# LiliMeng/network_interpretation_imagenet

Measured on NVIDIA B200. Metric: masked forward evals/sec (ResNet-101 224^2), higher is better.
Workload: dtype bf16

## Files before the change

network_interpretation_imagenet_b200/classifier.py:

```python
from __future__ import annotations

import ctypes as C

import numpy as np
import torch
import torch.nn as nn

from . import _lib


def _f32(t: torch.Tensor) -> np.ndarray:
    return np.ascontiguousarray(t.detach().to(torch.float32).cpu().numpy())


def fold_bn(conv_w: torch.Tensor, conv_b: torch.Tensor | None, bn: nn.BatchNorm2d | None):
    w = conv_w.detach().double()
    b = conv_b.detach().double() if conv_b is not None else torch.zeros(w.shape[0], dtype=torch.float64, device=w.device)
    if bn is not None:
        scale = bn.weight.detach().double() / torch.sqrt(bn.running_var.detach().double() + bn.eps)
        w = w * scale.view(-1, 1, 1, 1)
        b = bn.bias.detach().double() + (b - bn.running_mean.detach().double()) * scale
    elif conv_b is None:
        return w.float(), None
    return w.float(), b.float()
# ... 204 lines not shown
        buf = self.taps[name]
        H, W, Cc = C.c_int(), C.c_int(), C.c_int()
        _lib.check(self.lib.nib_net_buffer_info(self.h, buf, None, C.byref(H), C.byref(W), C.byref(Cc), None, None),
                   "nib_net_buffer_info")
        out = torch.empty(N, Cc.value, H.value, W.value, dtype=torch.float32, device="cuda")
        _lib.check(self.lib.nib_net_read_buffer_nchw(self.h, buf, N, out.data_ptr(), _lib.stream_handle()),
                   "nib_net_read_buffer_nchw")
        return out


def _in_cpad(Cin: int) -> int:
    return 4 if Cin <= 4 else Cin


def _lower_tv_resnet(m, hw, prec, precision, max_batch):
    H, W = hw
    b = _Builder(prec, max_batch)
    cin = m.conv1.in_channels
    c1 = m.conv1
    stem_tc = (precision == "bf16" and c1.kernel_size == (7, 7) and c1.stride == (2, 2) and c1.padding == (3, 3) and cin <= 8)
    split = precision == "split"
    x_in = (b.buffer(H, W, 4 if cin <= 4 else 8, pad=3, pooled=False) if stem_tc
            else b.buffer(H, W, _in_cpad(cin), pooled=False, f32=split))
    Hc, Wc = _out_hw(H, c1.kernel_size[0], c1.stride[0], c1.padding[0]), _out_hw(W, c1.kernel_size[0], c1.stride[0], c1.padding[0])
    t = b.buffer(Hc, Wc, c1.out_channels, f32=split)
    w, bias = fold_bn(c1.weight, c1.bias, m.bn1)
    b.conv(x_in, cin, t, c1.out_channels, w, bias, c1.kernel_size[0], c1.stride[0], c1.padding[0], relu=True)
    mp = m.maxpool
    k, s, p = mp.kernel_size, mp.stride, mp.padding
    Hp, Wp = _out_hw(Hc, k, s, p), _out_hw(Wc, k, s, p)
    x = b.buffer(Hp, Wp, c1.out_channels, f32=split)
    b.pool(_lib.POOL_MAX, t, c1.out_channels, x, k, s, p)
    b.release(t)
    if split:
        xs = b.buffer(Hp, Wp, c1.out_channels)
        b.convert(x, xs)
        b.release(x)
        x = xs
    Cx, Hx, Wx = c1.out_channels, Hp, Wp
    for layer in (m.layer1, m.layer2, m.layer3, m.layer4):
        for blk in layer:
            convs = [(blk.conv1, blk.bn1), (blk.conv2, blk.bn2)]
            if hasattr(blk, "conv3"):
                convs.append((blk.conv3, blk.bn3))
            if blk.downsample is not None:
                dc, dbn = blk.downsample[0], blk.downsample[1]
                Hd, Wd = _out_hw(Hx, dc.kernel_size[0], dc.stride[0], dc.padding[0]), _out_hw(Wx, dc.kernel_size[0], dc.stride[0], dc.padding[0])
                idn = b.buffer(Hd, Wd, dc.out_channels)
                w, bias = fold_bn(dc.weight, dc.bias, dbn)
                b.conv(x, Cx, idn, dc.out_channels, w, bias, dc.kernel_size[0], dc.stride[0], dc.padding[0], relu=False)
            else:
                idn = x
            cur, Cc, Hh, Ww = x, Cx, Hx, Wx
            tmp = []
            for i, (cv, bn) in enumerate(convs):
                last = i == len(convs) - 1
                Ho, Wo = _out_hw(Hh, cv.kernel_size[0], cv.stride[0], cv.padding[0]), _out_hw(Ww, cv.kernel_size[0], cv.stride[0], cv.padding[0])
                o = b.buffer(Ho, Wo, cv.out_channels)
                w, bias = fold_bn(cv.weight, cv.bias, bn)
                if last:
                    b.conv(cur, Cc, o, cv.out_channels, w, bias, cv.kernel_size[0], cv.stride[0], cv.padding[0],
                           relu=True, res=idn, res_C=cv.out_channels)
                else:
                    b.conv(cur, Cc, o, cv.out_channels, w, bias, cv.kernel_size[0], cv.stride[0], cv.padding[0], relu=True)
                    tmp.append(o)
                cur, Cc, Hh, Ww = o, cv.out_channels, Ho, Wo
            for tbuf in tmp:
                b.release(tbuf)
            if idn != x:
                b.release(idn)
            b.release(x)
            x, Cx, Hx, Wx = cur, Cc, Hh, Ww
    if split:
        xf = b.buffer(Hx, Wx, Cx, f32=True)
        b.convert(x, xf)
        x = xf
    feat = b.buffer(1, 1, Cx, f32=split)
    assert Hx == Wx, "global average pool expects a square map"
    b.pool(_lib.POOL_AVG, x, Cx, feat, Hx, Hx, 0)
    b.fc(feat, Cx, m.fc.out_features, m.fc.weight, m.fc.bias)
    return Classifier(b, x_in, (cin, H, W), m.fc.out_features, precision, max_batch, arch="tv_resnet")


def _lower_resnet_cifar(m, hw, prec, precision, max_batch):
    H, W = hw
    b = _Builder(prec, max_batch)
    cp = (lambda c: max(c, 64)) if precision == "bf16" else (lambda c: c)

    def padw(w, bias, co, ci):
        if co == w.shape[0] and ci == w.shape[1]:
            return w, bias
        wp = torch.zeros(co, ci, w.shape[2], w.shape[3], dtype=w.dtype, device=w.device)
        wp[:w.shape[0], :w.shape[1]] = w
        bp = None
        if bias is not None:
            bp = torch.zeros(co, dtype=bias.dtype, device=bias.device)
            bp[:bias.shape[0]] = bias
        return wp, bp

    x_in = b.buffer(H, W, _in_cpad(3), pooled=False)
    x = b.buffer(H, W, cp(16))
    w, bias = padw(*fold_bn(m.conv1.weight, None, m.bn1), cp(16), 3)
    b.conv(x_in, 3, x, cp(16), w, bias, 3, 1, 1, relu=True)
    Cx, Hx, Wx = 16, H, W
    for layer in (m.layer1, m.layer2, m.layer3):
        for blk in layer:
            s = blk.conv1.stride[0]
            planes = blk.conv1.out_channels
            Ho, Wo = _out_hw(Hx, 3, s, 1), _out_hw(Wx, 3, s, 1)
            t = b.buffer(Ho, Wo, cp(planes))
            w, bias = padw(*fold_bn(blk.conv1.weight, None, blk.bn1), cp(planes), cp(Cx))
            b.conv(x, cp(Cx), t, cp(planes), w, bias, 3, s, 1, relu=True)
            if blk.downsample is not None:
                ks = blk.downsample.avg.kernel_size
# ... 67 lines not shown
            b.release(mid)
            cur += c2.out_channels
        else:
            b.conv(blk_buf, cur, blk_buf, c1.out_channels, c1.weight.detach().float(), None, 3, 1, 1, relu=False,
                   out_coff=cur, pre=bn_affine(n1))
            cur += c1.out_channels
    assert cur == Ctot
    return cur


def _lower_tv_densenet(m, hw, prec, precision, max_batch):
    H, W = hw
    f = m.features
    b = _Builder(prec, max_batch)
    c0 = f.conv0
    stem_tc = (precision == "bf16" and c0.kernel_size == (7, 7) and c0.stride == (2, 2) and c0.padding == (3, 3))
    x_in = b.buffer(H, W, 4, pad=3, pooled=False) if stem_tc else b.buffer(H, W, _in_cpad(3), pooled=False)
    Hc, Wc = _out_hw(H, 7, 2, 3), _out_hw(W, 7, 2, 3)
    t = b.buffer(Hc, Wc, c0.out_channels)
    w, bias = fold_bn(c0.weight, None, f.norm0)
    b.conv(x_in, 3, t, c0.out_channels, w, bias, 7, 2, 3, relu=True)
    Hx, Wx = _out_hw(Hc, 3, 2, 1), _out_hw(Wc, 3, 2, 1)
    blocks = [getattr(f, n) for n in ("denseblock1", "denseblock2", "denseblock3", "denseblock4")]
    trans = [getattr(f, n) for n in ("transition1", "transition2", "transition3")]
    Cin = c0.out_channels
    prev, prev_is_stem = t, True
    for bi, blk in enumerate(blocks):
        layers = list(blk.children())
        growth = layers[0].conv2.out_channels
        Ctot = Cin + growth * len(layers)
        buf = b.buffer(Hx, Wx, Ctot, pooled=False)
        if prev_is_stem:
            b.pool(_lib.POOL_MAX, prev, Cin, buf, 3, 2, 1)
            b.release(prev)
        else:
            b.pool(_lib.POOL_AVG, prev, Cin, buf, 2, 2, 0)
            b.release(prev)
        _dense_block(b, layers, buf, Cin, Hx, Wx, Ctot)
        if bi < len(trans):
            tr = trans[bi]
            Co = tr.conv.out_channels
            tt = b.buffer(Hx, Wx, Co)
            b.conv(buf, Ctot, tt, Co, tr.conv.weight.detach().float(), None, 1, 1, 0, relu=False, pre=bn_affine(tr.norm))
            prev, prev_is_stem = tt, False
            Cin = Co
            Hx, Wx = Hx // 2, Wx // 2
        else:
            feat = b.buffer(1, 1, Ctot)
            assert Hx == Wx
            b.pool(_lib.POOL_AVG, buf, Ctot, feat, Hx, Hx, 0, pre=bn_affine(f.norm5))
            b.fc(feat, Ctot, m.classifier.out_features, m.classifier.weight, m.classifier.bias)
    return Classifier(b, x_in, (3, H, W), m.classifier.out_features, precision, max_batch, arch="tv_densenet")


def _lower_densenet_cifar(m, hw, prec, precision, max_batch):
    H, W = hw
    b = _Builder(prec, max_batch)
    x_in = b.buffer(H, W, _in_cpad(3), pooled=False)
    seq = list(m.blocks.children())
    Cin = m.stem.out_channels
    Hx, Wx = H, W
    prev = None
    for i in range(0, len(seq), 2):
        layers = list(seq[i].children())
        growth = (layers[0].conv2 if hasattr(layers[0], "conv2") else layers[0].conv1).out_channels
        Ctot = Cin + growth * len(layers)
        buf = b.buffer(Hx, Wx, Ctot, pooled=False)
        if prev is None:
            b.conv(x_in, 3, buf, Cin, m.stem.weight.detach().float(), None, 3, 1, 1, relu=False)
        else:
            b.pool(_lib.POOL_AVG, prev, Cin, buf, 2, 2, 0)
            b.release(prev)
        _dense_block(b, layers, buf, Cin, Hx, Wx, Ctot)
        if i + 1 < len(seq):
            tr = list(seq[i + 1].children())
            Co = tr[2].out_channels
            tt = b.buffer(Hx, Wx, Co)
            b.conv(buf, Ctot, tt, Co, tr[2].weight.detach().float(), None, 1, 1, 0, relu=False, pre=bn_affine(tr[0]))
            prev, Cin = tt, Co
            Hx, Wx = Hx // 2, Wx // 2
        else:
            feat = b.buffer(1, 1, Ctot)
            assert Hx == 8 and Wx == 8, "avg_pool2d(8) expects an 8x8 map (models/densenet.py:96)"
            b.pool(_lib.POOL_AVG, buf, Ctot, feat, 8, 8, 0, pre=bn_affine(m.norm5))
            b.fc(feat, Ctot, m.classifier.out_features, m.classifier.weight, m.classifier.bias)
# ... 2 lines not shown
```

network_interpretation_imagenet_b200/csrc/conv_tc.cu:

```cuda
#include "common.cuh"
#include "layers.cuh"
#include <cuda.h>
#include <string.h>
#include <stdlib.h>

namespace nib {

static constexpr int TC_BLOCK_M = 128;
static constexpr int TC_BLOCK_K = 64;
static constexpr int TC_UMMA_K = 16;
static constexpr int TC_THREADS = 192;

struct TcKernelParams {
  const float* bias;
  const __nv_bfloat16* res;
  void* out;
  int M;
  int Cout;
  int out_cstride, out_coff;
  int res_cstride, res_coff;
  int relu;
  int out_f32;
  int num_k_blocks;
  int cblocks;
  int S;
  int im2col;
  int tile_rows;
  int a_bytes;
  int P, Q, stride, pad;
  int in_coff;
  int n_tiles;
  int m_tiles;
  unsigned int* err_flag;
  unsigned long long* dbg;
  int a_wrap;
  int lo_off_out;
  int lo_off_res;
  const int* dyn_n;
  int halo_wp, halo_r, halo_tpi;
  int halo_cb, halo_n;
  const float* xf_scale;
  const float* xf_shift;
  int halo_swap;
};

__device__ __forceinline__ uint32_t smem_u32(const void* p) { return (uint32_t)__cvta_generic_to_shared(p); }

__device__ __forceinline__ void mbar_init(uint32_t bar, uint32_t count) {
  asm volatile("mbarrier.init.shared::cta.b64 [%0], %1;" ::"r"(bar), "r"(count) : "memory");
}
__device__ __forceinline__ void mbar_arrive_expect_tx(uint32_t bar, uint32_t bytes) {
  asm volatile("mbarrier.arrive.expect_tx.shared::cta.b64 _, [%0], %1;" ::"r"(bar), "r"(bytes) : "memory");
}
__device__ __forceinline__ bool mbar_try_wait(uint32_t bar, uint32_t parity) {
  uint32_t done;
  asm volatile(
      "{\n\t.reg .pred p;\n\t"
      "mbarrier.try_wait.parity.shared::cta.b64 p, [%1], %2;\n\t"
      "selp.u32 %0, 1, 0, p;\n\t}"
      : "=r"(done)
      : "r"(bar), "r"(parity)
      : "memory");
  return done != 0;
}
__device__ __forceinline__ void mbar_wait(uint32_t bar, uint32_t parity, unsigned int* err_flag, int code) {
  if (mbar_try_wait(bar, parity)) return;
  const long long t0 = clock64();
  while (!mbar_try_wait(bar, parity)) {
    if (clock64() - t0 > 4000000000LL) {
      if (err_flag) atomicExch(err_flag, (unsigned)code);
      __trap();
    }
  }
}
__device__ __forceinline__ void tma_load_2d(uint32_t dst, const CUtensorMap* tm, uint32_t bar, int c0, int c1) {
  asm volatile(
// ... 245 lines not shown
          *reinterpret_cast<float4*>(op + j) = make_float4(f[j], f[j + 1], f[j + 2], f[j + 3]);
      } else {
        __nv_bfloat16* op = reinterpret_cast<__nv_bfloat16*>(p.out) + (size_t)row * p.out_cstride + p.out_coff + col0;
#pragma unroll
        for (int j = 0; j < 32; j += 8) {
          uint4 o;
          __nv_bfloat162 h;
          h = __floats2bfloat162_rn(f[j], f[j + 1]);     o.x = *reinterpret_cast<uint32_t*>(&h);
          h = __floats2bfloat162_rn(f[j + 2], f[j + 3]); o.y = *reinterpret_cast<uint32_t*>(&h);
          h = __floats2bfloat162_rn(f[j + 4], f[j + 5]); o.z = *reinterpret_cast<uint32_t*>(&h);
          h = __floats2bfloat162_rn(f[j + 6], f[j + 7]); o.w = *reinterpret_cast<uint32_t*>(&h);
          *reinterpret_cast<uint4*>(op + j) = o;
        }
      }
      }
    }
    tc_fence_before();
  }
  __syncthreads();
  if (warp == 1) {
    tc_fence_after();
    asm volatile("tcgen05.dealloc.cta_group::1.sync.aligned.b32 %0, %1;" ::"r"(tmem_base),
                 "r"((uint32_t)(BLOCK_N < 32 ? 32 : BLOCK_N))
                 : "memory");
  }
}


__device__ __forceinline__ void mbar_arrive(uint32_t bar) {
  asm volatile("mbarrier.arrive.shared::cta.b64 _, [%0];" ::"r"(bar) : "memory");
}
__device__ __forceinline__ void tma_store_2d(const CUtensorMap* tm, uint32_t src, int c0, int c1) {
  asm volatile("cp.async.bulk.tensor.2d.global.shared::cta.bulk_group [%0, {%2, %3}], [%1];"
               ::"l"(reinterpret_cast<uint64_t>(tm)), "r"(src), "r"(c0), "r"(c1)
               : "memory");
}
__device__ __forceinline__ void bulk_commit() { asm volatile("cp.async.bulk.commit_group;" ::: "memory"); }
template <int N>
__device__ __forceinline__ void bulk_wait_read() { asm volatile("cp.async.bulk.wait_group.read %0;" ::"n"(N) : "memory"); }
__device__ __forceinline__ void fence_async_smem() { asm volatile("fence.proxy.async.shared::cta;" ::: "memory"); }
__device__ __forceinline__ uint4 lds_v4(uint32_t addr) {
  uint4 v;
  asm volatile("ld.shared.v4.u32 {%0,%1,%2,%3}, [%4];" : "=r"(v.x), "=r"(v.y), "=r"(v.z), "=r"(v.w) : "r"(addr));
  return v;
}
__device__ __forceinline__ void sts_v4(uint32_t addr, uint4 v) {
  asm volatile("st.shared.v4.u32 [%0], {%1,%2,%3,%4};" ::"r"(addr), "r"(v.x), "r"(v.y), "r"(v.z), "r"(v.w) : "memory");
}

static constexpr int TC3_THREADS = 64 + 256;
static constexpr int TC3_XF_WARPS = 4;
static constexpr int TC3_THREADS_XF = TC3_THREADS + 32 * TC3_XF_WARPS;

static constexpr int TC3_BRES_KBLOCKS = 9;
template <int BLOCK_N, int STAGES, bool HAS_RES, bool BRES = false, bool SPLIT = false>
struct Tc3Smem {
  static constexpr int A_BYTES = TC_BLOCK_M * TC_BLOCK_K * 2;
  static constexpr int BH_BYTES = (BLOCK_N / 2) * TC_BLOCK_K * 2;
  static constexpr int STAGE_BYTES = A_BYTES + (BRES ? 0 : BH_BYTES);
  static constexpr int BRES_BYTES = BRES ? TC3_BRES_KBLOCKS * BH_BYTES : 0;
  static constexpr int NBOX = BLOCK_N / 64;
  static constexpr bool SPLIT_COLS = NBOX >= 2;
  static constexpr int CW = SPLIT_COLS ? BLOCK_N / 2 : 64;
  static constexpr int UNITS = CW / 64;
  static constexpr int BOX_BYTES = TC_BLOCK_M * 128;
  static constexpr int RSETS = HAS_RES ? (BLOCK_N == 256 ? 1 : 2) : 1;
// ... 616 lines not shown
            sts_v4(obase_lo + ((((uint32_t)c) ^ sw) << 4), make_uint4(lo[c * 4], lo[c * 4 + 1], lo[c * 4 + 2], lo[c * 4 + 3]));
          fence_async_smem();
          __syncwarp();
          if (lane == 0) {
            tma_store_2d(&tmOut, slab_lo, p.out_coff + p.lo_off_out + n0 + b * 64, m0 + quarter * 32);
            bulk_commit();
            if (HAS_RES) {
              bulk_wait_read<0>();
              mbar_arrive(box_free_bar(buf));
              mbar_arrive(box_free_bar(buf_lo));
            }
          }
          continue;
        }
        uint32_t o[32];
        const uint32_t bsrc = bias_s + (uint32_t)(u * 64 * 4);
#pragma unroll
        for (int c = 0; c < 8; ++c) {
          uint64_t a0 = pack_f32x2(v[c * 8 + 0], v[c * 8 + 1]), a1 = pack_f32x2(v[c * 8 + 2], v[c * 8 + 3]);
          uint64_t a2 = pack_f32x2(v[c * 8 + 4], v[c * 8 + 5]), a3 = pack_f32x2(v[c * 8 + 6], v[c * 8 + 7]);
          if (has_bias) {
            const uint4 b0 = lds_v4(bsrc + (uint32_t)(c * 32)), b1 = lds_v4(bsrc + (uint32_t)(c * 32 + 16));
            a0 = add_f32x2(a0, pack_f32x2(b0.x, b0.y)); a1 = add_f32x2(a1, pack_f32x2(b0.z, b0.w));
            a2 = add_f32x2(a2, pack_f32x2(b1.x, b1.y)); a3 = add_f32x2(a3, pack_f32x2(b1.z, b1.w));
          }
          if (HAS_RES) {
            const uint4 r = lds_v4(obase + ((((uint32_t)c) ^ sw) << 4));
            a0 = add_f32x2(a0, pack_f32x2(r.x << 16, r.x & 0xFFFF0000u)); a1 = add_f32x2(a1, pack_f32x2(r.y << 16, r.y & 0xFFFF0000u));
            a2 = add_f32x2(a2, pack_f32x2(r.z << 16, r.z & 0xFFFF0000u)); a3 = add_f32x2(a3, pack_f32x2(r.w << 16, r.w & 0xFFFF0000u));
          }
          o[c * 4 + 0] = max_bf16x2(cvt_bf16x2(a0), relu_floor); o[c * 4 + 1] = max_bf16x2(cvt_bf16x2(a1), relu_floor);
          o[c * 4 + 2] = max_bf16x2(cvt_bf16x2(a2), relu_floor); o[c * 4 + 3] = max_bf16x2(cvt_bf16x2(a3), relu_floor);
        }
        if (halo) {
          if (quarter == 0 && lane == 0) TC3_TIMED(2, bulk_wait_read<0>());
          TC3_TIMED(3, named_bar_sync(1 + g, 128));
          if (halo_valid) {
#pragma unroll
            for (int c = 0; c < 8; ++c)
              if (c < 4 || p.halo_n == 64)
                sts_v4(halo_base + ((((uint32_t)c) ^ halo_sw) << 4), make_uint4(o[c * 4], o[c * 4 + 1], o[c * 4 + 2], o[c * 4 + 3]));
          }
          fence_async_smem();
          TC3_TIMED(3, named_bar_sync(1 + g, 128));
          if (quarter == 0 && lane == 0) {
            tma_store_2d(&tmOutTail, box_addr(g), p.out_coff + n0, m0);
            bulk_commit();
          }
          continue;
        }
        if (!HAS_RES) {
          if (lane == 0) TC3_TIMED(2, bulk_wait_read<0>());
          __syncwarp();
        }
#pragma unroll
        for (int c = 0; c < 8; ++c)
          sts_v4(obase + ((((uint32_t)c) ^ sw) << 4), make_uint4(o[c * 4], o[c * 4 + 1], o[c * 4 + 2], o[c * 4 + 3]));
        fence_async_smem();
        __syncwarp();
        if (lane == 0) {
          if (rows_here >= 32) tma_store_2d(&tmOut, slab, p.out_coff + n0 + b * 64, m0 + quarter * 32);
          else if (rows_here > 0) tma_store_2d(&tmOutTail, slab, p.out_coff + n0 + b * 64, m0 + quarter * 32);
          bulk_commit();
          if (HAS_RES) {
            if (u > 0) {
              TC3_TIMED(2, bulk_wait_read<1>());
// ... 401 lines not shown
                                    CUtensorMapSwizzle, CUtensorMapL2promotion, CUtensorMapFloatOOBfill);
typedef CUresult (*PFN_encodeIm2col)(CUtensorMap*, CUtensorMapDataType, cuuint32_t, void*, const cuuint64_t*,
                                     const cuuint64_t*, const int*, const int*, cuuint32_t, cuuint32_t,
                                     const cuuint32_t*, CUtensorMapInterleave, CUtensorMapSwizzle,
                                     CUtensorMapL2promotion, CUtensorMapFloatOOBfill);
static PFN_encodeTiled g_encodeTiled = nullptr;
static PFN_encodeIm2col g_encodeIm2col = nullptr;

static int load_driver_fns() {
  if (g_encodeTiled && g_encodeIm2col) return NIB_OK;
  cudaDriverEntryPointQueryResult q;
  void* fn = nullptr;
  NIB_CUDA(cudaGetDriverEntryPoint("cuTensorMapEncodeTiled", &fn, cudaEnableDefault, &q));
  if (q != cudaDriverEntryPointSuccess || !fn) { set_error("cuTensorMapEncodeTiled not available"); return NIB_ECUDA; }
  g_encodeTiled = (PFN_encodeTiled)fn;
  fn = nullptr;
  NIB_CUDA(cudaGetDriverEntryPoint("cuTensorMapEncodeIm2col", &fn, cudaEnableDefault, &q));
  if (q != cudaDriverEntryPointSuccess || !fn) { set_error("cuTensorMapEncodeIm2col not available"); return NIB_ECUDA; }
  g_encodeIm2col = (PFN_encodeIm2col)fn;
  return NIB_OK;
}

struct TcConvPlan {
  CUtensorMap tmA, tmB, tmOut, tmRes;
  CUtensorMap tmBh;
  CUtensorMap tmOut32, tmOutTail;
  int v3;
  int split;
  int block_n, stages;
  int im2col;
  int tile_rows;
  int num_k_blocks, cblocks;
  int halo_wp, halo_r, halo_tpi, halo_cb, halo_n;
  unsigned int* err_flag;
};

static unsigned int* g_err_flag = nullptr;

static int encode_2d_bf16(CUtensorMap* tm, const void* ptr, uint64_t inner, uint64_t outer, uint64_t row_bytes,
                          uint32_t box_inner, uint32_t box_outer) {
  cuuint64_t dims[2] = {inner, outer};
  cuuint64_t strides[1] = {row_bytes};
  cuuint32_t box[2] = {box_inner, box_outer};
  cuuint32_t es[2] = {1, 1};
  CUresult r = g_encodeTiled(tm, CU_TENSOR_MAP_DATA_TYPE_BFLOAT16, 2, const_cast<void*>(ptr), dims, strides, box, es,
                             CU_TENSOR_MAP_INTERLEAVE_NONE, CU_TENSOR_MAP_SWIZZLE_128B,
                             CU_TENSOR_MAP_L2_PROMOTION_L2_256B, CU_TENSOR_MAP_FLOAT_OOB_FILL_NONE);
  if (r != CUDA_SUCCESS) {
    set_error("cuTensorMapEncodeTiled failed (%d): dims=(%llu,%llu) row_bytes=%llu box=(%u,%u) ptr=%p", (int)r,
              (unsigned long long)inner, (unsigned long long)outer, (unsigned long long)row_bytes, box_inner,
              box_outer, ptr);
    return NIB_ECUDA;
  }
  return NIB_OK;
}

bool tc_conv_is_stem(const ConvParams& p) {
  return p.R == 7 && p.S == 7 && p.stride == 2 && p.pad == 3 && p.Cin <= 8 && p.in_cstride == 8 && p.in_coff == 0 &&
         p.in_halo == 3 && p.Cout % 32 == 0 && p.Q <= TC_BLOCK_M && p.out_halo == 0 && p.out_cstride % 8 == 0 &&
         p.out_coff % 8 == 0 && p.pre_scale == nullptr && p.res == nullptr && p.w_alt != nullptr &&
         (p.Win + 2 * p.in_halo) >= 2 * (p.Q - 1) + 8;
}

bool tc_conv_is_stem4(const ConvParams& p) {
  return p.R == 7 && p.S == 7 && p.stride == 2 && p.pad == 3 && p.Cin <= 4 && p.in_cstride == 4 &&
         p.in_coff == 0 && p.in_halo == 3 && p.Cout % 64 == 0 && p.Q <= TC_BLOCK_M && p.out_halo == 0 &&
// ... 123 lines not shown
        return NIB_ECUDA;
      }
    } else {
      cuuint64_t dims[4] = {32, (cuuint64_t)p.Q, (cuuint64_t)Hp, (cuuint64_t)max_batch};
      cuuint64_t strides[3] = {16, (cuuint64_t)Wp * 8, (cuuint64_t)Hp * Wp * 8};
      cuuint32_t box[4] = {32, (cuuint32_t)p.Q, 1, 1};
      cuuint32_t es[4] = {1, 1, 1, 1};
      CUresult r = g_encodeTiled(&plan->tmA, CU_TENSOR_MAP_DATA_TYPE_BFLOAT16, 4, const_cast<void*>(p.in), dims, strides,
                                 box, es, CU_TENSOR_MAP_INTERLEAVE_NONE, CU_TENSOR_MAP_SWIZZLE_64B,
                                 CU_TENSOR_MAP_L2_PROMOTION_L2_256B, CU_TENSOR_MAP_FLOAT_OOB_FILL_NONE);
      if (r != CUDA_SUCCESS) {
        set_error("cuTensorMapEncodeTiled (stem, 4-channel rows, 64B swizzle) failed (%d)", (int)r);
        delete plan;
        return NIB_ECUDA;
      }
    }
    rc = finish_plan(plan, p, max_batch, p.w_alt, 4 * 64);
    if (rc != NIB_OK) { delete plan; return rc; }
    {
      cuuint64_t dims[2] = {256, (cuuint64_t)p.Cout};
      cuuint64_t strides[1] = {256 * 2};
      cuuint32_t box[2] = {32, (cuuint32_t)(plan->block_n / 2)};
      cuuint32_t es[2] = {1, 1};
      CUresult r = g_encodeTiled(&plan->tmBh, CU_TENSOR_MAP_DATA_TYPE_BFLOAT16, 2, const_cast<void*>(p.w_alt), dims, strides,
                                 box, es, CU_TENSOR_MAP_INTERLEAVE_NONE, CU_TENSOR_MAP_SWIZZLE_64B,
                                 CU_TENSOR_MAP_L2_PROMOTION_L2_256B, CU_TENSOR_MAP_FLOAT_OOB_FILL_NONE);
      if (r != CUDA_SUCCESS) {
        set_error("cuTensorMapEncodeTiled (stem weights, 64B swizzle) failed (%d)", (int)r);
        delete plan;
        return NIB_ECUDA;
      }
    }
    plan->tmB = plan->tmBh;
    *out = plan;
    return NIB_OK;
  }
  if (tc_conv_is_stem(p)) {
    plan->im2col = 2;
    plan->cblocks = 1;
    plan->num_k_blocks = 7;
    plan->tile_rows = p.Q;
    rc = encode_2d_bf16(&plan->tmB, p.w_alt, 7 * 64, (uint64_t)p.Cout, 7 * 64 * 2, TC_BLOCK_K, plan->block_n);
    if (rc != NIB_OK) { delete plan; return rc; }
    const int Hp = p.Hin + 6, Wp = p.Win + 6;
    cuuint64_t dims[4] = {64, (cuuint64_t)p.Q, (cuuint64_t)Hp, (cuuint64_t)max_batch};
    cuuint64_t strides[3] = {32, (cuuint64_t)Wp * 16, (cuuint64_t)Hp * Wp * 16};
    cuuint32_t box[4] = {64, (cuuint32_t)p.Q, 1, 1};
    cuuint32_t es[4] = {1, 1, 1, 1};
    CUresult r = g_encodeTiled(&plan->tmA, CU_TENSOR_MAP_DATA_TYPE_BFLOAT16, 4, const_cast<void*>(p.in), dims, strides,
                               box, es, CU_TENSOR_MAP_INTERLEAVE_NONE, CU_TENSOR_MAP_SWIZZLE_128B,
                               CU_TENSOR_MAP_L2_PROMOTION_L2_256B, CU_TENSOR_MAP_FLOAT_OOB_FILL_NONE);
    if (r != CUDA_SUCCESS) {
      set_error("cuTensorMapEncodeTiled (stem, overlapping windows) failed (%d)", (int)r);
      delete plan;
      return NIB_ECUDA;
    }
    rc = finish_plan(plan, p, max_batch, p.w_alt, 7 * 64);
    if (rc != NIB_OK) { delete plan; return rc; }
    *out = plan;
    return NIB_OK;
  }
  if (tc_conv_is_halo3x3(p)) {
    const int Wp = p.Win + 2, R = halo_rows_per_tile(p.Hin, Wp);
    plan->im2col = 4;
    plan->cblocks = p.Cin / 64;
    plan->num_k_blocks = 9 * plan->cblocks;
// ... 233 lines not shown
    attr_set = true;
  }
  conv_tc_kernel<BLOCK_N, STAGES><<<tiles, TC_THREADS, SM::TOTAL, st>>>(plan->tmA, plan->tmB, kp);
  NIB_LAUNCH_CHECK();
  return NIB_OK;
}

template <int BLOCK_N, int STAGES, bool HAS_RES, bool BRES = false, bool SPLIT = false>
static int launch_tc3(const TcConvPlan* plan, const TcKernelParams& kp, cudaStream_t st) {
  using SM = Tc3Smem<BLOCK_N, STAGES, HAS_RES, BRES, SPLIT>;
  static_assert(SM::TOTAL <= 232448, "exceeds the 227 KB per-CTA shared memory limit");
  static bool attr_set = false;
  if (!attr_set) {
    NIB_CUDA(cudaFuncSetAttribute(conv_tc3_kernel<BLOCK_N, STAGES, HAS_RES, BRES, SPLIT>,
                                  cudaFuncAttributeMaxDynamicSharedMemorySize, SM::TOTAL));
    attr_set = true;
  }
  const int pair_tiles = ((kp.m_tiles + 1) / 2) * kp.n_tiles;
  const int max_pairs = num_sms() / 2;
  const int pairs = pair_tiles < max_pairs ? pair_tiles : max_pairs;
  static const bool pdl = getenv("NIB_TC_NO_PDL") == nullptr;
  cudaStreamCaptureStatus cap = cudaStreamCaptureStatusNone;
  cudaStreamIsCapturing(st, &cap);
  cudaLaunchConfig_t cfg;
  memset(&cfg, 0, sizeof(cfg));
  cfg.gridDim = dim3(2 * pairs);
  cfg.blockDim = dim3((!BRES && !SPLIT && kp.xf_scale != nullptr) ? TC3_THREADS_XF : TC3_THREADS);
  cfg.dynamicSmemBytes = SM::TOTAL;
  cfg.stream = st;
  cudaLaunchAttribute attr[1];
  attr[0].id = cudaLaunchAttributeProgrammaticStreamSerialization;
  attr[0].val.programmaticStreamSerializationAllowed = 1;
  cfg.attrs = attr;
  cfg.numAttrs = (pdl && cap == cudaStreamCaptureStatusNone && kp.dbg == nullptr) ? 1 : 0;
  NIB_CUDA(cudaLaunchKernelEx(&cfg, conv_tc3_kernel<BLOCK_N, STAGES, HAS_RES, BRES, SPLIT>, plan->tmA, plan->tmBh, plan->tmOut32,
                              plan->tmOutTail, plan->tmRes, kp));
  return NIB_OK;
}

static int tc_dispatch(const TcConvPlan* plan, const TcKernelParams& kp, int tiles, cudaStream_t st) {
  if (plan->split) {
    const bool res = kp.res != nullptr;
    if (!plan->v3 || kp.out_f32) { set_error("tc_dispatch: split mode needs the CTA-pair kernel"); return NIB_EINVAL; }
    if (plan->block_n == 256) return res ? launch_tc3<256, 3, true, false, true>(plan, kp, st) : launch_tc3<256, 6, false, false, true>(plan, kp, st);
    if (plan->block_n == 128) return res ? launch_tc3<128, 4, true, false, true>(plan, kp, st) : launch_tc3<128, 8, false, false, true>(plan, kp, st);
    return res ? launch_tc3<64, 8, true, false, true>(plan, kp, st) : launch_tc3<64, 9, false, false, true>(plan, kp, st);
  }
  if (plan->v3 && !kp.out_f32) {
    const bool res = kp.res != nullptr;
    if (plan->im2col == 4) return launch_tc3<64, 9, false, true>(plan, kp, st);
    if (plan->block_n == 256) return res ? launch_tc3<256, 5, true>(plan, kp, st) : launch_tc3<256, 6, false>(plan, kp, st);
    if (plan->block_n == 128) return res ? launch_tc3<128, 6, true>(plan, kp, st) : launch_tc3<128, 8, false>(plan, kp, st);
    if (plan->block_n == 64 && !res && kp.n_tiles == 1 && kp.num_k_blocks <= TC3_BRES_KBLOCKS)
      return launch_tc3<64, 9, false, true>(plan, kp, st);
    if (plan->block_n == 64) return res ? launch_tc3<64, 9, true>(plan, kp, st) : launch_tc3<64, 9, false>(plan, kp, st);
  }
  switch (plan->block_n) {
    case 32:  return launch_tc<32, 4>(plan, kp, tiles, st);
    case 64:  return launch_tc<64, 4>(plan, kp, tiles, st);
    case 128: return launch_tc<128, 3>(plan, kp, tiles, st);
    case 256: return launch_tc<256, 4>(plan, kp, tiles, st);
  }
  set_error("tc_dispatch: bad block_n %d", plan->block_n);
  return NIB_EINVAL;
}

static int tc_launch_debug(const TcConvPlan* plan, TcKernelParams kp, const ConvParams& p, int tiles, cudaStream_t st) {
// ... 67 lines not shown
  kp.P = p.P;
  kp.Q = p.Q;
  kp.stride = p.stride;
  kp.pad = p.pad;
  kp.in_coff = p.in_coff;
  kp.n_tiles = ceil_div(p.Cout, plan->block_n);
  kp.err_flag = plan->err_flag;
  kp.tile_rows = plan->tile_rows;
  kp.a_bytes = plan->tile_rows * TC_BLOCK_K * 2;
  kp.m_tiles = ceil_div(p.M, plan->tile_rows);
  kp.a_wrap = plan->split ? 2 * p.Cin / TC_BLOCK_K : plan->cblocks;
  kp.lo_off_out = p.out_lo_off;
  kp.lo_off_res = p.res_lo_off;
  kp.dyn_n = plan->split ? p.dyn_n : nullptr;
  if (p.pre_scale != nullptr) {
    if (!(p.pre_padded && plan->im2col == 0 && plan->v3 && !plan->split)) {
      set_error("tc_conv_launch: a pre-activation conv reached a tensor path without the transform role");
      return NIB_EINVAL;
    }
    kp.xf_scale = p.pre_scale;
    kp.xf_shift = p.pre_shift;
  }
  if (plan->im2col == 4) {
    kp.n_tiles = 1;
    kp.halo_cb = plan->halo_cb; kp.halo_n = plan->halo_n;
    kp.halo_wp = plan->halo_wp; kp.halo_r = plan->halo_r; kp.halo_tpi = plan->halo_tpi;
    kp.a_bytes = (plan->halo_r + 2) * plan->halo_wp * 128;
  }
  if (plan->im2col == 5) {
    static const bool swap = getenv("NIB_TC_STEM_SWAP") != nullptr;
    kp.halo_wp = plan->halo_wp;
    kp.halo_swap = swap ? 1 : 0;
    kp.a_bytes = 7 * plan->halo_wp;
  }
  const int tiles = kp.m_tiles * kp.n_tiles;
  static const bool dbg = getenv("NIB_TC_DBG") != nullptr;
  if (dbg && plan->v3) return tc_launch_debug(plan, kp, p, tiles, st);
  return tc_dispatch(plan, kp, tiles, st);
}

}

extern "C" int nib_tc_gemm_bf16(const void* d_A, const void* d_B, float* d_C, int M, int N, int K, void* stream) {
  NIB_DEVICE_OR_FAIL();
  using namespace nib;
  NIB_REQUIRE(d_A && d_B && d_C, "nib_tc_gemm_bf16: null pointer");
  NIB_REQUIRE(M > 0 && N > 0 && K > 0 && K % 64 == 0 && N % 32 == 0, "nib_tc_gemm_bf16: need K%%64==0, N%%32==0");
  int rc = load_driver_fns();
  if (rc != NIB_OK) return rc;
  if (!g_err_flag) {
    NIB_CUDA(cudaMalloc(&g_err_flag, sizeof(unsigned int)));
    NIB_CUDA(cudaMemset(g_err_flag, 0, sizeof(unsigned int)));
  }
  TcConvPlan plan;
  memset(&plan, 0, sizeof(plan));
  plan.err_flag = g_err_flag;
  plan.block_n = pick_block_n(N);
  plan.cblocks = K / TC_BLOCK_K;
  plan.num_k_blocks = plan.cblocks;
  plan.im2col = 0;
  rc = encode_2d_bf16(&plan.tmB, d_B, (uint64_t)K, (uint64_t)N, (uint64_t)K * 2, TC_BLOCK_K, plan.block_n);
  if (rc != NIB_OK) return rc;
  rc = encode_2d_bf16(&plan.tmA, d_A, (uint64_t)K, (uint64_t)M, (uint64_t)K * 2, TC_BLOCK_K, TC_BLOCK_M);
  if (rc != NIB_OK) return rc;
  TcKernelParams kp;
  memset(&kp, 0, sizeof(kp));
// ... 17 lines not shown
```

network_interpretation_imagenet_b200/csrc/layers.cuh:

```cuda
#pragma once
#include "common.cuh"

namespace nib {

struct ConvParams {
  const void* in;
  const void* w;
  const void* w_alt;
  const float* bias;
  const void* res;
  void* out;
  const float* pre_scale;
  const float* pre_shift;
  int pre_padded;
  int M;
  int Hin, Win, Cin, in_cstride, in_coff, in_halo;
  int P, Q, Cout, out_cstride, out_coff, out_halo;
  int res_cstride, res_coff, res_C;
  int R, S, stride, pad;
  int relu;
  const int* dyn_n;
  int split;
  int in_lo_off, out_lo_off, res_lo_off;
};

struct PoolParams {
  const void* in;
  void* out;
  const float* pre_scale;
  const float* pre_shift;
  int kind, N, Hin, Win, C, in_cstride, in_coff;
  int P, Q, out_cstride, out_coff;
  int k, stride, pad;
  const int* dyn_n;
};

int launch_conv_simt(const ConvParams& p, bool bf16, cudaStream_t st);
bool conv_x3_supported(const ConvParams& p);
int launch_conv_x3(const ConvParams& p, const void* w_hi, const void* w_lo, cudaStream_t st);
int launch_pool(const PoolParams& p, bool bf16, cudaStream_t st);
bool fc_x2_supported(int Cin, int feat_stride);
int launch_fc_x2(const void* feat, int feat_stride, const void* w_hi, const void* w_lo, const float* b, int N, int Cin,
                 int Cout, float* logits, const int* dyn_n, cudaStream_t st);
int launch_fc(const void* feat, int feat_stride, bool bf16, const float* w, const float* b, int N, int Cin,
              int Cout, float* logits, const int* dyn_n, cudaStream_t st);
int launch_bnrelu_pack(const void* x, int in_cstride, int in_coff, int Cin, int Cpad, const float* scale,
                       const float* shift, void* y, long long M, cudaStream_t st);
int launch_nchw_to_nhwc(const float* x, int N, int C, int H, int W, void* out, int cs, int halo, bool bf16,
                        cudaStream_t st);
int launch_nhwc_to_nchw(const void* in, int N, int C, int H, int W, int cs, int halo, bool bf16, float* out,
                        cudaStream_t st);
int launch_split_convert(const void* in, void* out, long long M, int C, bool to_split, const int* dyn_n, int rows_per_image,
                         cudaStream_t st);
int mask_synth_impl(const nib_mask_args* a, cudaStream_t st, bool skip_halo, const int* dyn_n = nullptr);

struct TcConvPlan;
// ... 15 lines not shown
```

network_interpretation_imagenet_b200/csrc/net.cu:

```cuda
#include "common.cuh"
#include "layers.cuh"
#include <vector>
#include <map>
#include <string.h>

using namespace nib;

enum BufKind { BUF_F32 = 0, BUF_BF16 = 1, BUF_SPLIT = 2 };

struct NetBuffer {
  int H, W, C, pad;
  int kind;
  void* ptr;
  size_t elems_per_image;
  int phys_c() const { return kind == BUF_SPLIT ? 2 * C : C; }
  size_t esize() const { return kind == BUF_F32 ? 4 : 2; }
};

struct NetOp {
  int kind;
  nib_conv_desc cd;
  void* d_w;
  void* d_w_alt;
  float* d_bias;
  float* d_pre_scale;
  float* d_pre_shift;
  void* d_w_pack;
  int pack_cin;
  float* d_pre_scale_pad;
  float* d_pre_shift_pad;
  int xform;
  void* d_w_hi;
  void* d_w_lo;
  TcConvPlan* plan;
  TcFusedPlan* fplan;
  bool fused_skip;
  nib_conv_desc next_cd;
  void* next_w;
  float* next_bias;
  int pool_kind, k, stride, pad, C, in_buf, in_coff, out_buf, out_coff;
  int fc_in, fc_cin, fc_cout;
};

struct nib_net {
  int precision;
  int max_batch;
  bool bf16;
  bool x3;
  bool split;
  std::vector<NetBuffer> bufs;
  std::vector<NetOp> ops;
  void* pack_scratch;
  size_t pack_scratch_bytes;
  int input_buf;
  bool finalized;
  int num_classes;
  bool use_tc;
  bool use_graph;
  const int* dyn_n;
  long long launches, tc_launches, x3_launches;
  static constexpr size_t kMaxGraphs = 8;
  struct GraphVal { cudaGraphExec_t exec; long long launches, tc_launches; };
  std::map<int, GraphVal> graphs;
  float* graph_logits;
};

static size_t elem_size(const nib_net* n) { return n->bf16 ? 2 : 4; }

static int upload_floats(const float* h, size_t n, float** d) {
  *d = nullptr;
  if (!h || n == 0) return NIB_OK;
  NIB_CUDA(cudaMalloc(d, n * sizeof(float)));
// ... 305 lines not shown
  net->input_buf = buf;
  return NIB_OK;
}

static void fill_conv_params(const nib_net* net, const NetOp& op, int N, ConvParams* p) {
  const nib_conv_desc& d = op.cd;
  const NetBuffer& bi = net->bufs[d.in_buf];
  const NetBuffer& bo = net->bufs[d.out_buf];
  memset(p, 0, sizeof(*p));
  p->in = bi.ptr;
  p->w = op.d_w;
  p->w_alt = op.d_w_alt;
  p->bias = op.d_bias;
  p->out = bo.ptr;
  p->pre_scale = op.d_pre_scale;
  p->pre_shift = op.d_pre_shift;
  p->Hin = bi.H; p->Win = bi.W; p->Cin = d.Cin; p->in_cstride = bi.phys_c(); p->in_coff = d.in_coff; p->in_halo = bi.pad;
  p->P = bo.H; p->Q = bo.W; p->Cout = d.Cout; p->out_cstride = bo.phys_c(); p->out_coff = d.out_coff; p->out_halo = bo.pad;
  p->split = bi.kind == BUF_SPLIT ? 1 : 0;
  p->in_lo_off = bi.C;
  p->out_lo_off = bo.C;
  p->M = N * bo.H * bo.W;
  if (d.res_buf >= 0) {
    const NetBuffer& br = net->bufs[d.res_buf];
    p->res = br.ptr;
    p->res_cstride = br.phys_c(); p->res_coff = d.res_coff; p->res_C = d.res_C;
    p->res_lo_off = br.C;
  }
  p->R = d.R; p->S = d.S; p->stride = d.stride; p->pad = d.pad;
  p->relu = (d.flags & NIB_CONV_RELU) ? 1 : 0;
  p->dyn_n = net->dyn_n;
}

static void fill_xform_conv_params(const nib_net* net, const NetOp& op, int N, ConvParams* p) {
  fill_conv_params(net, op, N, p);
  p->w = op.d_w_pack;
  p->pre_scale = op.d_pre_scale_pad;
  p->pre_shift = op.d_pre_shift_pad;
  p->pre_padded = 1;
  p->Cin = op.pack_cin;
}

static void fill_packed_conv_params(const nib_net* net, const NetOp& op, int N, ConvParams* p) {
  fill_conv_params(net, op, N, p);
  p->in = net->pack_scratch;
  p->w = op.d_w_pack;
  p->pre_scale = nullptr;
  p->pre_shift = nullptr;
  p->Cin = op.pack_cin;
  p->in_cstride = op.pack_cin;
  p->in_coff = 0;
}

int nib_net_finalize(nib_net* net) {
  NIB_REQUIRE(net && !net->finalized, "nib_net_finalize: bad handle/state");
  NIB_REQUIRE(net->input_buf >= 0, "nib_net_finalize: input buffer not set");
  NIB_REQUIRE(!net->ops.empty() && net->ops.back().kind == 2, "nib_net_finalize: the last op must be the fc layer");
  if (net->split) {
    for (auto& op : net->ops) {
      if (op.kind != 0 || net->bufs[op.cd.in_buf].kind != BUF_SPLIT) continue;
      ConvParams p;
      fill_conv_params(net, op, net->max_batch, &p);
      NIB_REQUIRE(tc_conv_supported(p), "nib_net_finalize: a conv on split tensors needs Cin %% 64 == 0, Cout %% 64 == 0, whole-buffer channel ranges (Cin=%d Cout=%d)", p.Cin, p.Cout);
      int rc = tc_conv_plan_create(p, net->max_batch, &op.plan);
      if (rc != NIB_OK) return rc;
    }
// ... 12 lines not shown
      if (need > net->pack_scratch_bytes) net->pack_scratch_bytes = need;
    }
    if (net->pack_scratch_bytes) NIB_CUDA(cudaMalloc(&net->pack_scratch, net->pack_scratch_bytes + 256));
    for (auto& op : net->ops) {
      if (op.kind != 0) continue;
      ConvParams p;
      if (op.xform) {
        fill_xform_conv_params(net, op, net->max_batch, &p);
        int rc = tc_conv_plan_create(p, net->max_batch, &op.plan);
        if (rc != NIB_OK) return rc;
        continue;
      }
      if (op.pack_cin) {
        fill_packed_conv_params(net, op, net->max_batch, &p);
        if (tc_conv_supported(p)) {
          int rc = tc_conv_plan_create(p, net->max_batch, &op.plan);
          if (rc != NIB_OK) return rc;
        } else {
          op.pack_cin = 0;
        }
        continue;
      }
      fill_conv_params(net, op, net->max_batch, &p);
      if (tc_conv_supported(p)) {
        int rc = tc_conv_plan_create(p, net->max_batch, &op.plan);
        if (rc != NIB_OK) {
          if (op.d_w_alt == nullptr) return rc;
          op.plan = nullptr;
        }
      }
    }
  }
  if (net->bf16) {
    for (size_t i = 0; i + 1 < net->ops.size(); ++i) {
      NetOp& c = net->ops[i];
      NetOp& a = net->ops[i + 1];
      if (c.kind != 0 || a.kind != 0 || !c.plan || !a.plan || c.pack_cin || a.pack_cin || c.fused_skip) continue;
      ConvParams pc, pa;
      fill_conv_params(net, c, net->max_batch, &pc);
      fill_conv_params(net, a, net->max_batch, &pa);
      if (!tc_fuse_supported(pc, pa)) continue;
      int rc = tc_fused_plan_create(pc, pa, net->max_batch, &c.fplan);
      if (rc != NIB_OK) return rc;
      c.next_cd = a.cd;
      c.next_w = a.d_w;
      c.next_bias = a.d_bias;
      a.fused_skip = true;
    }
  }
  net->finalized = true;
  return NIB_OK;
}

static int run_ops(nib_net* net, int N, float* d_logits, cudaStream_t st) {
  for (auto& op : net->ops) {
    if (op.kind == 0) {
      if (op.fused_skip && net->use_tc) continue;
      ConvParams p;
      fill_conv_params(net, op, N, &p);
      int rc;
      if (op.fplan && net->use_tc) {
        NetOp nx = op;
        nx.cd = op.next_cd;
        nx.d_w = op.next_w;
        nx.d_bias = op.next_bias;
        ConvParams pa;
        fill_conv_params(net, nx, N, &pa);
        rc = tc_fused_launch(op.fplan, p, pa, st);
        net->tc_launches++;
      } else if (op.plan && net->use_tc && op.xform) {
        fill_xform_conv_params(net, op, N, &p);
        rc = tc_conv_launch(op.plan, p, st);
        net->tc_launches++;
      } else if (op.plan && net->use_tc && op.pack_cin) {
        const NetBuffer& bi = net->bufs[op.cd.in_buf];
        rc = launch_bnrelu_pack(bi.ptr, bi.C, op.cd.in_coff, op.cd.Cin, op.pack_cin, op.d_pre_scale, op.d_pre_shift,
                                net->pack_scratch, (long long)N * bi.H * bi.W, st);
        net->launches++;
        if (rc != NIB_OK) return rc;
        fill_packed_conv_params(net, op, N, &p);
        rc = tc_conv_launch(op.plan, p, st);
        net->tc_launches++;
      } else if (op.plan && (net->use_tc || net->split)) {
        rc = tc_conv_launch(op.plan, p, st);
        net->tc_launches++;
      } else if (net->x3 && op.d_w_hi && conv_x3_supported(p)) {
        rc = launch_conv_x3(p, op.d_w_hi, op.d_w_lo, st);
        net->x3_launches++;
      } else {
        rc = launch_conv_simt(p, net->bf16, st);
      }
      net->launches++;
      if (rc != NIB_OK) return rc;
    } else if (op.kind == 3) {
      const NetBuffer& bi = net->bufs[op.in_buf];
      const NetBuffer& bo = net->bufs[op.out_buf];
      int rc = launch_split_convert(bi.ptr, bo.ptr, (long long)N * bi.H * bi.W, bi.C, bi.kind == BUF_F32, net->dyn_n, bi.H * bi.W, st);
      net->launches++;
      if (rc != NIB_OK) return rc;
    } else if (op.kind == 1) {
      const NetBuffer& bi = net->bufs[op.in_buf];
      const NetBuffer& bo = net->bufs[op.out_buf];
      PoolParams p;
      memset(&p, 0, sizeof(p));
      p.in = bi.ptr; p.out = bo.ptr;
      p.pre_scale = op.d_pre_scale; p.pre_shift = op.d_pre_shift;
      p.kind = op.pool_kind; p.N = N; p.Hin = bi.H; p.Win = bi.W; p.C = op.C;
      p.in_cstride = bi.C; p.in_coff = op.in_coff;
      p.P = bo.H; p.Q = bo.W; p.out_cstride = bo.C; p.out_coff = op.out_coff;
      p.k = op.k; p.stride = op.stride; p.pad = op.pad;
      p.dyn_n = net->dyn_n;
      int rc = launch_pool(p, bi.kind == BUF_BF16, st);
      net->launches++;
      if (rc != NIB_OK) return rc;
    } else {
      const NetBuffer& bi = net->bufs[op.fc_in];
      static const bool fc_simt = getenv("NIB_FC_SIMT") != nullptr;
      int rc = (op.d_w_hi && !fc_simt)
                   ? launch_fc_x2(bi.ptr, bi.C, op.d_w_hi, op.d_w_lo, op.d_bias, N, op.fc_cin, op.fc_cout, d_logits, net->dyn_n, st)
                   : launch_fc(bi.ptr, bi.C, bi.kind == BUF_BF16, (const float*)op.d_w, op.d_bias, N, op.fc_cin, op.fc_cout,
                               d_logits, net->dyn_n, st);
      net->launches++;
      if (rc != NIB_OK) return rc;
    }
  }
  return NIB_OK;
}

static int stage_input(nib_net* net, const void* d_x, int x_layout, int N, cudaStream_t st) {
  const NetBuffer& bi = net->bufs[net->input_buf];
  NIB_REQUIRE(bi.kind != BUF_SPLIT, "nib_net_forward: the input buffer of a split network must be fp32 (nib_net_add_buffer_f32)");
  if (x_layout == NIB_IN_NCHW_F32) {
    int C = bi.C;
// ... 196 lines not shown
```

Before: 45290.

## Fuse stem conv with 3x3/2 max pool via TMA max-reduce stores

The bf16 7x7 stem conv epilogue now computes a horizontal 3-wide max in registers with warp shuffles and neighbour-quarter edge exchange in shared memory. It then issues TMA max-reduce bulk stores into the pooled output, one or two pooled rows per conv row, so the separate max-pool launch and the full-resolution stem activation write and read are skipped. In exchange the pooled buffer must be zeroed with a memset each launch, which relies on ReLU outputs being non-negative. PDL is also disabled for this launch, and a fallback env switch is added. Taps are plumbed in Python, apparently for interpretability access to the pooled map.

Result: no change. 45580 (median of 6 runs) (+0.6%).

```diff
diff --git a/network_interpretation_imagenet_b200/classifier.py b/network_interpretation_imagenet_b200/classifier.py
--- a/network_interpretation_imagenet_b200/classifier.py
+++ b/network_interpretation_imagenet_b200/classifier.py
@@ -260,6 +260,7 @@
     x = b.buffer(Hp, Wp, c1.out_channels, f32=split)
     b.pool(_lib.POOL_MAX, t, c1.out_channels, x, k, s, p)
     b.release(t)
+    taps = {"pool": x}
     if split:
         xs = b.buffer(Hp, Wp, c1.out_channels)
         b.convert(x, xs)
@@ -307,7 +308,7 @@
     assert Hx == Wx, "global average pool expects a square map"
     b.pool(_lib.POOL_AVG, x, Cx, feat, Hx, Hx, 0)
     b.fc(feat, Cx, m.fc.out_features, m.fc.weight, m.fc.bias)
-    return Classifier(b, x_in, (cin, H, W), m.fc.out_features, precision, max_batch, arch="tv_resnet")
+    return Classifier(b, x_in, (cin, H, W), m.fc.out_features, precision, max_batch, taps=taps, arch="tv_resnet")
 
 
 def _lower_resnet_cifar(m, hw, prec, precision, max_batch):
@@ -441,6 +442,7 @@
         buf = b.buffer(Hx, Wx, Ctot, pooled=False)
         if prev_is_stem:
             b.pool(_lib.POOL_MAX, prev, Cin, buf, 3, 2, 1)
+            taps = {"pool0": buf}
             b.release(prev)
         else:
             b.pool(_lib.POOL_AVG, prev, Cin, buf, 2, 2, 0)
@@ -459,7 +461,7 @@
             assert Hx == Wx
             b.pool(_lib.POOL_AVG, buf, Ctot, feat, Hx, Hx, 0, pre=bn_affine(f.norm5))
             b.fc(feat, Ctot, m.classifier.out_features, m.classifier.weight, m.classifier.bias)
-    return Classifier(b, x_in, (3, H, W), m.classifier.out_features, precision, max_batch, arch="tv_densenet")
+    return Classifier(b, x_in, (3, H, W), m.classifier.out_features, precision, max_batch, taps=taps, arch="tv_densenet")
 
 
 def _lower_densenet_cifar(m, hw, prec, precision, max_batch):
diff --git a/network_interpretation_imagenet_b200/csrc/conv_tc.cu b/network_interpretation_imagenet_b200/csrc/conv_tc.cu
--- a/network_interpretation_imagenet_b200/csrc/conv_tc.cu
+++ b/network_interpretation_imagenet_b200/csrc/conv_tc.cu
@@ -42,6 +42,7 @@
   const float* xf_scale;
   const float* xf_shift;
   int halo_swap;
+  int pool_p, pool_q, pool_coff;
 };
 
 __device__ __forceinline__ uint32_t smem_u32(const void* p) { return (uint32_t)__cvta_generic_to_shared(p); }
@@ -353,6 +354,11 @@
 }
 __device__ __forceinline__ void tma_store_2d(const CUtensorMap* tm, uint32_t src, int c0, int c1) {
   asm volatile("cp.async.bulk.tensor.2d.global.shared::cta.bulk_group [%0, {%2, %3}], [%1];"
+               ::"l"(reinterpret_cast<uint64_t>(tm)), "r"(src), "r"(c0), "r"(c1)
+               : "memory");
+}
+__device__ __forceinline__ void tma_reduce_max_2d(const CUtensorMap* tm, uint32_t src, int c0, int c1) {
+  asm volatile("cp.reduce.async.bulk.tensor.2d.global.shared::cta.max.tile.bulk_group [%0, {%2, %3}], [%1];"
                ::"l"(reinterpret_cast<uint64_t>(tm)), "r"(src), "r"(c0), "r"(c1)
                : "memory");
 }
@@ -1035,6 +1041,51 @@
           o[c * 4 + 0] = max_bf16x2(cvt_bf16x2(a0), relu_floor); o[c * 4 + 1] = max_bf16x2(cvt_bf16x2(a1), relu_floor);
           o[c * 4 + 2] = max_bf16x2(cvt_bf16x2(a2), relu_floor); o[c * 4 + 3] = max_bf16x2(cvt_bf16x2(a3), relu_floor);
         }
+        if (BRES && !HAS_RES && !SPLIT && p.pool_p > 0) {
+          const uint32_t box = box_addr(g);
+          const uint32_t edge = box + (uint32_t)p.pool_q * 128u;
+          if (quarter == 0 && lane == 0) TC3_TIMED(2, bulk_wait_read<0>());
+          TC3_TIMED(3, named_bar_sync(1 + g, 128));
+          if (lane == 31) {
+#pragma unroll
+            for (int c = 0; c < 8; ++c)
+              sts_v4(edge + (uint32_t)quarter * 128u + (uint32_t)c * 16u, make_uint4(o[c * 4], o[c * 4 + 1], o[c * 4 + 2], o[c * 4 + 3]));
+          }
+#pragma unroll
+          for (int k = 0; k < 32; ++k) {
+            const uint32_t x = o[k];
+            const uint32_t left = __shfl_up_sync(0xffffffffu, x, 1), right = __shfl_down_sync(0xffffffffu, x, 1);
+            o[k] = max_bf16x2(x, right);
+            if (lane > 0) o[k] = max_bf16x2(o[k], left);
+          }
+          const int j = quarter * 16 + (lane >> 1);
+          const bool owner = (lane & 1) == 0 && j < p.pool_q;
+          const uint32_t orow = box + (uint32_t)j * 128u;
+          if (owner) {
+#pragma unroll
+            for (int c = 0; c < 8; ++c) sts_v4(orow + (uint32_t)c * 16u, make_uint4(o[c * 4], o[c * 4 + 1], o[c * 4 + 2], o[c * 4 + 3]));
+          }
+          TC3_TIMED(3, named_bar_sync(1 + g, 128));
+          if (owner && lane == 0 && quarter > 0) {
+#pragma unroll
+            for (int c = 0; c < 8; ++c) {
+              const uint4 e = lds_v4(edge + (uint32_t)(quarter - 1) * 128u + (uint32_t)c * 16u);
+              const uint4 v = lds_v4(orow + (uint32_t)c * 16u);
+              sts_v4(orow + (uint32_t)c * 16u, make_uint4(max_bf16x2(v.x, e.x), max_bf16x2(v.y, e.y), max_bf16x2(v.z, e.z),
+                                                          max_bf16x2(v.w, e.w)));
+            }
+          }
+          fence_async_smem();
+          TC3_TIMED(3, named_bar_sync(1 + g, 128));
+          if (quarter == 0 && lane == 0) {
+            const int img = m_tile / p.P, r = m_tile - img * p.P;
+            const int row0 = img * p.pool_p * p.pool_q;
+            tma_reduce_max_2d(&tmRes, box, p.pool_coff, row0 + (r >> 1) * p.pool_q);
+            if ((r & 1) && (r >> 1) + 1 < p.pool_p) tma_reduce_max_2d(&tmRes, box, p.pool_coff, row0 + ((r >> 1) + 1) * p.pool_q);
+            bulk_commit();
+          }
+          continue;
+        }
         if (halo) {
           if (quarter == 0 && lane == 0) TC3_TIMED(2, bulk_wait_read<0>());
           TC3_TIMED(3, named_bar_sync(1 + g, 128));
@@ -1502,6 +1553,7 @@
   int tile_rows;
   int num_k_blocks, cblocks;
   int halo_wp, halo_r, halo_tpi, halo_cb, halo_n;
+  int pool;
   unsigned int* err_flag;
 };
 
@@ -1691,6 +1743,28 @@
       }
     }
     plan->tmB = plan->tmBh;
+    if (p.pool_out != nullptr) {
+      if (plan->im2col != 5 || !plan->v3 || p.Cout != 64 || p.relu == 0 || p.Q % 2 != 0 || p.pool_Q > 64 || p.pool_P != (p.P - 1) / 2 + 1 ||
+          p.pool_Q != (p.Q - 1) / 2 + 1 || p.pool_cstride % 8 != 0 || p.pool_coff % 8 != 0) {
+        set_error("tc_conv_plan_create: the stem + max pool launch needs the raw-row stem with 64 ReLU outputs");
+        delete plan;
+        return NIB_EINVAL;
+      }
+      const uint64_t rows = (uint64_t)max_batch * p.pool_P * p.pool_Q;
+      cuuint64_t dims[2] = {(cuuint64_t)p.pool_cstride, rows};
+      cuuint64_t strides[1] = {(cuuint64_t)p.pool_cstride * 2};
+      cuuint32_t box[2] = {64, (cuuint32_t)p.pool_Q};
+      cuuint32_t es[2] = {1, 1};
+      CUresult r = g_encodeTiled(&plan->tmRes, CU_TENSOR_MAP_DATA_TYPE_BFLOAT16, 2, p.pool_out, dims, strides, box, es,
+                                 CU_TENSOR_MAP_INTERLEAVE_NONE, CU_TENSOR_MAP_SWIZZLE_NONE,
+                                 CU_TENSOR_MAP_L2_PROMOTION_L2_256B, CU_TENSOR_MAP_FLOAT_OOB_FILL_NONE);
+      if (r != CUDA_SUCCESS) {
+        set_error("cuTensorMapEncodeTiled (stem pooled output) failed (%d)", (int)r);
+        delete plan;
+        return NIB_ECUDA;
+      }
+      plan->pool = 1;
+    }
     *out = plan;
     return NIB_OK;
   }
@@ -1990,7 +2064,7 @@
   attr[0].id = cudaLaunchAttributeProgrammaticStreamSerialization;
   attr[0].val.programmaticStreamSerializationAllowed = 1;
   cfg.attrs = attr;
-  cfg.numAttrs = (pdl && cap == cudaStreamCaptureStatusNone && kp.dbg == nullptr) ? 1 : 0;
+  cfg.numAttrs = (pdl && cap == cudaStreamCaptureStatusNone && kp.dbg == nullptr && kp.pool_p == 0) ? 1 : 0;
   NIB_CUDA(cudaLaunchKernelEx(&cfg, conv_tc3_kernel<BLOCK_N, STAGES, HAS_RES, BRES, SPLIT>, plan->tmA, plan->tmBh, plan->tmOut32,
                               plan->tmOutTail, plan->tmRes, kp));
   return NIB_OK;
@@ -2124,6 +2198,16 @@
     kp.halo_wp = plan->halo_wp;
     kp.halo_swap = swap ? 1 : 0;
     kp.a_bytes = 7 * plan->halo_wp;
+    if (plan->pool) {
+      if (p.pool_out == nullptr) { set_error("tc_conv_launch: a stem + max pool plan launched without its pooled output"); return NIB_EINVAL; }
+      kp.pool_p = p.pool_P;
+      kp.pool_q = p.pool_Q;
+      kp.pool_coff = p.pool_coff;
+      const size_t rows = (size_t)(p.M / (p.P * p.Q)) * p.pool_P * p.pool_Q;
+      char* base = static_cast<char*>(p.pool_out) + (size_t)p.pool_coff * 2;
+      if (p.pool_cstride == p.Cout) NIB_CUDA(cudaMemsetAsync(base, 0, rows * p.Cout * 2, st));
+      else NIB_CUDA(cudaMemset2DAsync(base, (size_t)p.pool_cstride * 2, 0, (size_t)p.Cout * 2, rows, st));
+    }
   }
   const int tiles = kp.m_tiles * kp.n_tiles;
   static const bool dbg = getenv("NIB_TC_DBG") != nullptr;
diff --git a/network_interpretation_imagenet_b200/csrc/layers.cuh b/network_interpretation_imagenet_b200/csrc/layers.cuh
--- a/network_interpretation_imagenet_b200/csrc/layers.cuh
+++ b/network_interpretation_imagenet_b200/csrc/layers.cuh
@@ -22,6 +22,8 @@
   const int* dyn_n;
   int split;
   int in_lo_off, out_lo_off, res_lo_off;
+  void* pool_out;
+  int pool_cstride, pool_coff, pool_P, pool_Q;
 };
 
 struct PoolParams {
diff --git a/network_interpretation_imagenet_b200/csrc/net.cu b/network_interpretation_imagenet_b200/csrc/net.cu
--- a/network_interpretation_imagenet_b200/csrc/net.cu
+++ b/network_interpretation_imagenet_b200/csrc/net.cu
@@ -38,6 +38,8 @@
   nib_conv_desc next_cd;
   void* next_w;
   float* next_bias;
+  bool stem_pool;
+  int stem_pool_buf, stem_pool_coff;
   int pool_kind, k, stride, pad, C, in_buf, in_coff, out_buf, out_coff;
   int fc_in, fc_cin, fc_cout;
 };
@@ -409,6 +411,14 @@
   p->dyn_n = net->dyn_n;
 }
 
+static void fill_stem_pool_params(const nib_net* net, const NetOp& op, int N, ConvParams* p) {
+  fill_conv_params(net, op, N, p);
+  const NetBuffer& bp = net->bufs[op.stem_pool_buf];
+  p->pool_out = bp.ptr;
+  p->pool_cstride = bp.C; p->pool_coff = op.stem_pool_coff;
+  p->pool_P = bp.H; p->pool_Q = bp.W;
+}
+
 static void fill_xform_conv_params(const nib_net* net, const NetOp& op, int N, ConvParams* p) {
   fill_conv_params(net, op, N, p);
   p->w = op.d_w_pack;
@@ -487,6 +497,25 @@
     }
   }
   if (net->bf16) {
+    const bool no_stem_pool = getenv("NIB_TC_NO_STEM_POOL") != nullptr;
+    for (size_t i = 0; i + 1 < net->ops.size() && !no_stem_pool; ++i) {
+      NetOp& c = net->ops[i];
+      NetOp& pl = net->ops[i + 1];
+      if (c.kind != 0 || !c.plan || !c.d_w_alt || c.pack_cin || pl.kind != 1 || pl.pool_kind != NIB_POOL_MAX) continue;
+      if (pl.k != 3 || pl.stride != 2 || pl.pad != 1 || pl.d_pre_scale || pl.in_buf != c.cd.out_buf ||
+          pl.in_coff != c.cd.out_coff || pl.C != c.cd.Cout || !(c.cd.flags & NIB_CONV_RELU))
+        continue;
+      c.stem_pool_buf = pl.out_buf;
+      c.stem_pool_coff = pl.out_coff;
+      ConvParams p;
+      fill_stem_pool_params(net, c, net->max_batch, &p);
+      TcConvPlan* fp = nullptr;
+      if (tc_conv_plan_create(p, net->max_batch, &fp) != NIB_OK) continue;
+      tc_conv_plan_destroy(c.plan);
+      c.plan = fp;
+      c.stem_pool = true;
+      pl.fused_skip = true;
+    }
     for (size_t i = 0; i + 1 < net->ops.size(); ++i) {
       NetOp& c = net->ops[i];
       NetOp& a = net->ops[i + 1];
@@ -512,7 +541,8 @@
     if (op.kind == 0) {
       if (op.fused_skip && net->use_tc) continue;
       ConvParams p;
-      fill_conv_params(net, op, N, &p);
+      if (op.stem_pool && net->use_tc) fill_stem_pool_params(net, op, N, &p);
+      else fill_conv_params(net, op, N, &p);
       int rc;
       if (op.fplan && net->use_tc) {
         NetOp nx = op;
@@ -554,6 +584,7 @@
       net->launches++;
       if (rc != NIB_OK) return rc;
     } else if (op.kind == 1) {
+      if (op.fused_skip && net->use_tc) continue;
       const NetBuffer& bi = net->bufs[op.in_buf];
       const NetBuffer& bo = net->bufs[op.out_buf];
       PoolParams p;
```
